# 10XGenomics/lariat

Measured on AMD Instinct MI355X. Metric: read-pairs/sec aligned to hg38 (per-barcode align loop: SMEM seeding + SW + RFA/MAPQ on device); synthetic hg38-scale reference, higher is better.
Workload: dtype u64/i32 (FM-index + integer DP), f64 (RFA scores)

## Files before the change

### lariat_amd/csrc/k_smem4.h

```cpp
#pragma once
#ifndef LH_K1_SLAB_CHUNK
#define LH_K1_SLAB_CHUNK 4
#endif
#include "lh_dev.h"
static_assert((LH_MAXLEN + 2) % LH_K1_SLAB_CHUNK == 0, "a lane's list of LH_MAXLEN + 2 entries is a whole number of chunks");

struct __attribute__((aligned(16))) PEnt { u64 lo, hi; };
#define LH_M40 0xffffffffffull
__device__ __forceinline__ PEnt pe_pack(u64 x0, u64 x1, u64 x2, int info) {
    PEnt e;
    e.lo = x0 | (x2 << 40);
    e.hi = x1 | ((x2 >> 24) << 40) | ((u64)(uint32_t)info << 49);
    return e;
}
#define PE_X0(e) ((e).lo & LH_M40)
#define PE_X1(e) ((e).hi & LH_M40)
#define PE_X2(e) (((e).lo >> 40) | ((((e).hi >> 40) & 0x1ffull) << 24))
#define PE_INFO(e) ((int)((e).hi >> 49))
#define LH_POSF (1ull << 62)

#define S4_FETCH 0
#define S4_DONE 1
#define S4_REQ_FWD 2
#define S4_REQ_BWD 3
// ... 136 lines not shown
#define K1T_BLOOM2 3
#define K1T_REPT 4
#define K1T_PLCP 5
#define K1T_TEXT 6
#define K1T_SA 7
#define K1T_ISA 8
#define K1T_SLAB_R 9
#define K1T_SLAB_W 10
#define K1T_INTV_W 11
#define K1T_READS 12
#define K1T_N 13
#ifdef LH_K1_TRACE
__device__ u64* lh_k1_trace;
__device__ uint32_t lh_k1_trace_cap;
__device__ uint32_t* lh_k1_trace_n;
#define K1_REQ(tab_, ptr_, bytes_)                                                                                                              \
    {                                                                                                                                            \
        if (PASS == 1 && !BIG && lh_k1_trace) {                                                                                                  \
            if (trace_k < lh_k1_trace_cap) lh_k1_trace[(size_t)trace_k * T + t] = (u64)(uintptr_t)(ptr_) | (u64)(bytes_) << 48 | (u64)(tab_) << 56; \
            ++trace_k;                                                                                                                           \
        }                                                                                                                                        \
    }
#else
#define K1_REQ(tab_, ptr_, bytes_)
#endif

template <int PASS, bool BIG>
__global__ void __launch_bounds__(64, PASS == 3 ? 8 : LH_SMEM4_WAVES) k_smem_pass(DIndex ix, DOpts o, int n_reads_all, const uint8_t* __restrict__ seq, const i64* __restrict__ seq_off,
                                               DIntv* __restrict__ intv_out, int32_t* __restrict__ n_intv, int32_t* __restrict__ status, PEnt* __restrict__ slab,
                                               int32_t* __restrict__ next_read, DCounters* __restrict__ ctr, K1Big big) {
    const int n_reads = (BIG || big.list) ? *big.count : n_reads_all;
    constexpr int ICAP = BIG ? LH_BIG_INTV : LH_MAX_INTV;
    __shared__ uint32_t qn[32 * 64];
    constexpr bool DO1 = PASS == 1, DO2 = PASS == 2, DO12 = DO1 || DO2, DO3 = PASS == 3, P3T = PASS == 3;
    const bool P2TASK = PASS == 2 && !BIG && big.list != nullptr;
    int task_k = 0;
    const bool P3TEXT = P3T && ix.isa != nullptr && ix.plcp != nullptr && o.max_mem_intv > 1;
    const int Lw = o.min_seed_len + 1;
    uint32_t uspan = 0;
#define P3_NOTEXT (1 << 30)
    u64 up0 = 0, up1 = 0;
#define US0 ((int)(uspan & 0xff))
#define UE0 ((int)((uspan >> 8) & 0xff))
#define US1 ((int)((uspan >> 16) & 0xff))
#define UE1 ((int)(uspan >> 24))
    const int lane = LANE();
    const uint32_t T = gridDim.x * 64u, t = blockIdx.x * 64u + (uint32_t)lane;
#ifdef LH_K1_TRACE
    uint32_t trace_k = 0;
// ... 39 lines not shown
#define RF_TRIF 128
    int todo = 0;
#define CODE16(s_, out_)                                                                                     \
    {                                                                                                        \
        uint32_t a_, b_;                                                                                     \
        Q8(s_, a_) Q8((s_) + 8, b_)                                                                          \
        a_ &= 0x33333333u; b_ &= 0x33333333u;                                                                \
        a_ = (a_ | a_ >> 2) & 0x0f0f0f0fu; a_ = (a_ | a_ >> 4) & 0x00ff00ffu; a_ = (a_ | a_ >> 8) & 0xffffu; \
        b_ = (b_ | b_ >> 2) & 0x0f0f0f0fu; b_ = (b_ | b_ >> 4) & 0x00ff00ffu; b_ = (b_ | b_ >> 8) & 0xffffu; \
        out_ = a_ | b_ << 16;                                                                                \
    }
#define QB(i_) ((int)((qn[((i_) >> 3) * 64 + lane] >> (((i_) & 7) * 4)) & 0xF))
#define Q8(s_, out_)                                                                                         \
    {                                                                                                        \
        int w_ = (s_) >> 3, sh_ = ((s_) & 7) * 4;                                                            \
        uint32_t lo_ = (w_ >= 0 && w_ < 32) ? qn[w_ * 64 + lane] : 0x44444444u;                              \
        uint32_t hi_ = (w_ + 1 >= 0 && w_ + 1 < 32) ? qn[(w_ + 1) * 64 + lane] : 0x44444444u;                \
        out_ = sh_ ? (lo_ >> sh_) | (hi_ << (32 - sh_)) : lo_;                                               \
    }
#define T16_LOAD(p_) { i64 w_ = (p_) >> 3; tw_sh = (uint32_t)((p_) & 7) * 4; tw0 = ix.tn[w_]; tw1 = ix.tn[w_ + 1]; tw2 = ix.tn[w_ + 2]; K1_REQ(K1T_TEXT, ix.tn + w_, 12) }
#define T16_A() (tw_sh ? (tw0 >> tw_sh) | (tw1 << (32 - tw_sh)) : tw0)
#define T16_B() (tw_sh ? (tw1 >> tw_sh) | (tw2 << (32 - tw_sh)) : tw1)
#define CURR ((rflags & RF_CURA) ? LA : LB)
#define PREV ((rflags & RF_CURA) ? LB : LA)
#define K1_SLAB_IX(e_) (((uint32_t)(e_) / LH_K1_SLAB_CHUNK) * (LH_K1_SLAB_CHUNK * T) + ((uint32_t)(e_) % LH_K1_SLAB_CHUNK))
#define PREV_AT(e_) PREV[K1_SLAB_IX(e_)]
#define FWD_ADVANCE()                                                                                        \
    {                                                                                                        \
        int b_ = i < len ? QB(i) : 4;                                                                        \
        if (b_ > 3) {       \
            ce = pe_pack(c0, c1, c2, cinfo);         \
            ncurr++;                                                                                         \
            st = S4_BWD_INIT;                                                                                \
        } else { ec = 3 - b_; st = S4_REQ_FWD; }                                                             \
    }
#define BLOOM_ISSUE()                                                                                        \
    {                                                                                                        \
        bword = 0; bmask = filt ? 1 : 0;    \
        if (pbits && cinfo - x <= LH_BLOOM_K) bword = (pbits >> (cinfo - x - 1)) & 1;    \
        else if (filt && cinfo >= filt_from) {                                                               \
            uint32_t w_;                                                                                     \
// ... 55 lines not shown
    }
#define BWD_ROW_BODY()                                                                                       \
    {                                                                                                        \
        int c_ = i < 0 ? 4 : QB(i);                                                                          \
        ncurr = 0; last_size = 0; j = 0;                                                                     \
        c0 = PE_X0(ce); c1 = PE_X1(ce); c2 = PE_X2(ce); cinfo = PE_INFO(ce);                                 \
        if (c_ > 3) {                  \
            if ((rflags & (RF_C1UNK | RF_RUNP)) == (RF_C1UNK | RF_RUNP)) { c0 = LH_POSF | (u64)run_p; c1 = 0; }    \
            st = S4_BWD_EMIT0;                                                                               \
        }                                                                                                    \
        else if (runs && nprev == 1 && c2 == 1 && min_intv == 1) { rflags &= ~RF_TRI; st = S4_BRUN_INIT; }    \
          \
        else if (by_text && (rflags & (RF_REV | RF_TRIF)) == RF_REV && nprev > 1 && c2 == 1 && min_intv == 1) { rflags |= RF_TRI; st = S4_BRUN_INIT; } \
        else {                                                                                               \
            ec = c_; st = S4_REQ_BWD;                                                                        \
            if (nprev > 1) { pn = PREV_AT((rflags & RF_REV) ? nprev - 2 : 1); K1_REQ(K1T_SLAB_R, &PREV_AT((rflags & RF_REV) ? nprev - 2 : 1), 16) }                                                \
            if (ktl) CODE16(i, rcode)                                                                        \
        }                                                                                                    \
    }
#define BWD_ADVANCE()                                                                                        \
    {                                                                                                        \
        ++j;                                                                                                 \
        if (j < nprev) {                                                                                     \
            c0 = PE_X0(pn); c1 = PE_X1(pn); c2 = PE_X2(pn); cinfo = PE_INFO(pn);                             \
            st = S4_REQ_BWD;                                                                                 \
            if (j + 1 < nprev) { pn = PREV_AT((rflags & RF_REV) ? nprev - 2 - j : j + 1); K1_REQ(K1T_SLAB_R, &PREV_AT((rflags & RF_REV) ? nprev - 2 - j : j + 1), 16) }                                    \
        } else if (ncurr == 0) st = S4_SMEM_DONE;                                                            \
        else {                                                                                               \
            nprev = ncurr; --i;                                                                              \
            rflags = (rflags ^ RF_CURA) & ~(RF_RUNP | RF_C1UNK | RF_REV);    \
            if (i < -1) st = S4_SMEM_DONE;                                                                   \
            else { todo |= TD_ROW; st = S4_PENDING; }                                                        \
        }                                                                                                    \
    }
#define EMIT_MEM()                                                                                           \
    {                                                                                                        \
        if (cinfo - (i + 1) >= o.min_seed_len) {                                                             \
            DIntv m_; m_.x0 = c0; m_.x1 = c1; m_.x2 = c2; m_.info = (u64)(uint32_t)cinfo | (u64)(i + 1) << 32;  \
            if (P2TASK) {        \
                const int slot_ = atomicAdd(&n_intv[r], 1);                                                  \
                if (slot_ >= ICAP) ovf = 1; else out[slot_] = m_;                                            \
// ... 4 lines not shown
    }
    for (;;) {
        const bool slow_turn = __popcll(__ballot(st == S4_FETCH || (st >= 8 && st < S4_FRUN_INIT))) >= (PASS == 3 ? LH_SLOW_BATCH_P3 : PASS == 2 ? LH_SLOW_BATCH_P2 : LH_SLOW_BATCH) ||
                               !__any((st >= S4_REQ_FWD && st < 8) || st >= S4_FRUN_INIT);
        u64 need = slow_turn ? __ballot(st == S4_FETCH) : 0;
        if (need) {
            int cnt = __popcll(need), newbase = 0;
            if (chunk_next + cnt > chunk_end) {
                int nb = 0;
                if (lane == 0) nb = atomicAdd(next_read, 64);
                newbase = wave_readlane(nb, 0);
            }
            i64 off = 0;
            int ln = 0, rr = -1;
            if (st == S4_FETCH) {
                int idx = chunk_next + lanes_below(need, lane);
                rr = idx < chunk_end ? idx : newbase + (idx - chunk_end);
                if (rr >= n_reads) st = S4_DONE;
                else {
                    if (BIG || big.list) rr = big.list[rr];
                    if (P2TASK) { task_k = rr & 15; rr >>= 4; }
                    off = seq_off[rr]; ln = (int)(seq_off[rr + 1] - off);
                }
            }
            if (chunk_next + cnt > chunk_end) { chunk_next = newbase + (chunk_next + cnt - chunk_end); chunk_end = newbase + 64; }
            else chunk_next += cnt;
            u64 got = __ballot(st == S4_FETCH);
            while (got) {
                int Lk[4], lnk[4];
                uint32_t wk[4];
                for (int k = 0; k < 4; ++k) {
// ... 4 lines not shown
                        const i64 offL = shfl_i64(off, Lk[k]);
                        lnk[k] = wave_readlane(ln, Lk[k]);
                        if (lnk[k] > LH_MAXLEN) lnk[k] = 0;
                        if (4 * lane < lnk[k]) __builtin_memcpy(&wk[k], seq + offL + 4 * lane, 4);
                    }
                }
                for (int k = 0; k < 4; ++k) {
                    if (Lk[k] < 0) break;
                    uint32_t nb16 = 0;
                    for (int b = 0; b < 4; ++b) {
                        uint32_t v = (wk[k] >> (8 * b)) & 0xff;
                        v = (4 * lane + b < lnk[k] && v < 4) ? v : 4;
                        nb16 |= v << (4 * b);
                    }
                    uint32_t other = __shfl_xor(nb16, 1);
                    if (!(lane & 1)) qn[(lane >> 1) * 64 + Lk[k]] = nb16 | other << 16;
                }
            }
            if (st == S4_FETCH) {
                r = rr; len = ln; rst = 0; on = 0; ovf = 0; p2mask = 0; rflags = 0;
                K1_REQ(K1T_READS, seq + off, 64)
                K1_REQ(K1T_READS, seq_off + rr, 16)
                if (len > LH_MAXLEN) { rst |= LH_ST_TOO_LONG; len = 0; }
                out = BIG ? big.slab + (size_t)big.slot[r] * (2 * LH_BIG_INTV) : intv_out + (size_t)r * LH_MAX_INTV;
                if (!DO1) { on = n_intv[r]; rst |= status[r]; }
                if (len >= o.min_seed_len) { x = 0; st = DO1 ? S4_P1_SCAN : DO2 ? S4_P2_NEXT : S4_P3_SCAN; }
                else st = S4_READ_DONE;
                if (DO1 && !BIG && big.resume) {
                    const K1Resume rs = big.resume[r];
                    if (rs.x > 0 && st == S4_P1_SCAN) {
                        x = rs.x; on = n_intv[r]; SET_X_PREV(((rs.pk >> 8) & 0xff) - 2); SET_BT_SKIP(((rs.pk >> 16) & 0xff) - 1);
// ... 312 lines not shown
            const u64 xb = isb ? c1 : c0;
            u64 s0 = tl[0] - tk[0], s1 = tl[1] - tk[1], s2 = tl[2] - tk[2], s3 = tl[3] - tk[3];
            u64 acc = xb + ((xa <= ix.primary && xa + c2 - 1 >= ix.primary) ? 1 : 0);
            u64 o3 = acc, o2 = o3 + s3, o1 = o2 + s2, o0 = o1 + s1;
            u64 na = ec == 0 ? ix.L2[0] + 1 + tk[0] : ec == 1 ? ix.L2[1] + 1 + tk[1] : ec == 2 ? ix.L2[2] + 1 + tk[2] : ix.L2[3] + 1 + tk[3];
            u64 nb = ec == 0 ? o0 : ec == 1 ? o1 : ec == 2 ? o2 : o3;
            ok.x2 = ec == 0 ? s0 : ec == 1 ? s1 : ec == 2 ? s2 : s3;
            if (isb) { ok.x0 = na; ok.x1 = nb; } else { ok.x1 = na; ok.x0 = nb; }
            n_exec_total++;
        }
        if (req) n_ext_total++;
        if (DO12 && st == S4_REQ_FWD) {
            if (ok.x2 != c2) {
                ce = pe_pack(c0, c1, c2, cinfo);
                if (ok.x2 < (u64)min_intv) { st = S4_BWD_INIT; ncurr++; }
                else if (FWD_PUSH_OK()) { if (!ncurr) emin = cinfo; CURR[K1_SLAB_IX(ncurr)] = ce; K1_REQ(K1T_SLAB_W, &CURR[K1_SLAB_IX(ncurr)], 16) ncurr++; }
            }
            if (st == S4_REQ_FWD) {
                c0 = ok.x0; c1 = ok.x1; c2 = ok.x2; cinfo = i + 1; ++i;
                wkey = wkey >> 2 | (u64)(3 - ec) << (2 * LH_BLOOM_K - 2);
                if (runs && c2 == 1 && min_intv == 1) st = S4_FRUN_INIT;
                else { todo |= TD_FADV; st = S4_PENDING; }
            }
        } else if (DO12 && st == S4_REQ_BWD) {
            if (ok.x2 < (u64)min_intv) {
                if (ncurr == 0 && (last_mem_start < 0 || i + 1 < last_mem_start)) st = S4_BWD_EMIT;
            } else if (ncurr == 0 || ok.x2 != last_size) {
                PEnt e = pe_pack(ok.x0, ok.x1, ok.x2, cinfo);
                if (ncurr == 0) ce = e;
                else { CURR[K1_SLAB_IX(ncurr)] = e; K1_REQ(K1T_SLAB_W, &CURR[K1_SLAB_IX(ncurr)], 16) }
                ncurr++;
                last_size = ok.x2;
            }
            if (st == S4_REQ_BWD) BWD_ADVANCE()
        } else if (DO1 && st == S4_REQ_FRUN) {
            uint32_t qa, qb;
            Q8(i, qa)
            Q8(i + 8, qb)
            uint32_t xa = qa ^ T16_A(), xb = qb ^ T16_B();
            int n = xa ? (__ffs((int)xa) - 1) >> 2 : 8 + (xb ? (__ffs((int)xb) - 1) >> 2 : 8);
            if (!(rflags & RF_BT)) n_ext_total += (unsigned)n;
            i += n;
            if (n == 16) T16_LOAD(run_p + (i - x))
            else if (rflags & RF_BT) {
                if (ec < i - x) {
// ... 35 lines not shown
            } else {
                c0 = ok.x0; c1 = ok.x1; c2 = ok.x2; ++i;
                P3_ADVANCE()
            }
        }
    }
#undef QB
#undef Q8
#undef CODE16
#undef T16_LOAD
#undef T16_A
#undef T16_B
#undef CURR
#undef PREV
#undef PREV_AT
#undef K1_SLAB_IX
#undef P3_NOTEXT
#undef US0
#undef UE0
#undef US1
#undef UE1
#undef START_SMEM1
#undef WKEY_AT
#undef BLOOM_ISSUE
#undef FWD_PUSH_OK
#undef FWD_ADVANCE
#undef P3_ADVANCE
#undef BWD_ROW_BODY
#undef BWD_ADVANCE
#undef EMIT_MEM
// ... 37 lines not shown
            const u64 e = trace[(size_t)k * T + t];
            const int tab = (int)(e >> 56), bytes = (int)((e >> 48) & 0xff);
            const uintptr_t a = (uintptr_t)(e & 0xffffffffffffull) + (acc == 0x9e3779b97f4a7c15ull ? 64 : 0);
            if (tab == K1T_SLAB_W) {
                uint4 v = {(uint32_t)acc, 1, 2, 3};
                *(uint4*)a = v;
            } else if (bytes >= 32) { const uint4 v0 = ((const uint4*)a)[0], v1 = ((const uint4*)a)[1]; acc += v0.x + v1.w; }
            else if (bytes >= 16) { const uint4 v = *(const uint4*)a; acc += v.x + v.w; }
            else if (bytes == 12) { const uint32_t* q = (const uint32_t*)a; acc += q[0] + q[1] + q[2]; }
            else if (bytes == 8) acc += *(const u64*)a;
            else acc += *(const uint8_t*)a;
        }
    }
    if (acc == 0x9e3779b97f4a7c15ull) *sink = acc;
}
__global__ void __launch_bounds__(256) k_k1_trace_hist(const u64* __restrict__ trace, const uint32_t* __restrict__ n_req, uint32_t cap, uint32_t T, unsigned long long* __restrict__ hist) {
    __shared__ unsigned long long h[2 * K1T_N + 2];
    if (threadIdx.x < 2 * K1T_N + 2) h[threadIdx.x] = 0;
    __syncthreads();
    for (uint32_t t = blockIdx.x * blockDim.x + threadIdx.x; t < T; t += gridDim.x * blockDim.x) {
        uint32_t n = n_req[t];
        if (n > cap) { atomicAdd(&h[2 * K1T_N], (unsigned long long)(n - cap)); n = cap; }
        for (uint32_t k = 0; k < n; ++k) {
            const u64 e = trace[(size_t)k * T + t];
            const int tab = (int)(e >> 56);
            if (tab < K1T_N) { atomicAdd(&h[2 * tab], 1ull); atomicAdd(&h[2 * tab + 1], (unsigned long long)((e >> 48) & 0xff)); }
        }
    }
    __syncthreads();
    if (threadIdx.x < 2 * K1T_N + 2 && h[threadIdx.x]) atomicAdd(&hist[threadIdx.x], h[threadIdx.x]);
// ... 239 lines not shown
```

### lariat_amd/csrc/lh_host.inc

```
#include <math.h>
#include <stdlib.h>
#include <stdio.h>
#include <string.h>

#include <functional>
#include <memory>
#include <mutex>
#include <string>
#include <vector>
#include <map>

#include "../../include/lariat_hip.h"
#include "k_smem4.h"
#include "k_chain_lane.h"
#include "k_chain_cl.h"
#include "k_rfa.h"
#include "k_rescue3.h"

#define LH_RFA_FIELDS DInf S; uint8_t* d_slab = nullptr; i64 slab_bytes = 0; int grid_rfa = 0; int32_t* d_bc_next = nullptr; \
    uint8_t* d_slab2 = nullptr; i64 slab2_bytes = 0; int grid_rfa2 = 0; uint8_t* d_slab_mid[2] = {nullptr, nullptr}; i64 slab_mid_bytes[2] = {0, 0}; int grid_rfa_mid[2] = {0, 0}; int grid_rfa_mid_max[2] = {0, 0}; int32_t* d_rfa_ovf_mid = nullptr;  int32_t* d_rfa_ovf = nullptr; int32_t* d_rfa_order = nullptr; int32_t *d_rfa_ovf2 = nullptr, *d_rfa_hp = nullptr, *d_rfa_hr = nullptr; double* d_bc_lmp = nullptr;

#define LH_STAGE2_FIELDS                                                                                         \
    i64* d_reg_off = nullptr; DReg* d_regs = nullptr; DReg* d_regs_tmp = nullptr; int32_t* d_ia = nullptr;        \
    int32_t* d_n_regs = nullptr; int32_t* d_best = nullptr; uint8_t* d_zpool = nullptr;                           \
// ... 52 lines not shown
    hipStream_t stream = nullptr;
    hipStream_t aux[3] = {nullptr, nullptr, nullptr};
    hipStream_t dl_stream = nullptr, up_stream = nullptr;
    hipEvent_t ev_pack = nullptr, ev_dl = nullptr;
    bool dl_pending = false, dl_split = false; std::function<int(lh_result**)> dl_finish;
    int sel_slot = 0;
    i64* h_peek = nullptr;
    bool ext_hint_valid = false;
    hipEvent_t ev_fork = nullptr, ev_join[3] = {nullptr, nullptr, nullptr};
    i64 cap_pairs = 0, cap_reads = 0, cap_bases = 0, pool_cap = 0, regpool_cap = 0, cap_bc = 0;
    int grid_smem4 = 0; PEnt* d_slab4 = nullptr; int32_t* d_next_read = nullptr;
    uint32_t* d_seq4 = nullptr;
    uint8_t* d_seq = nullptr; i64* d_seq_off = nullptr; u64* d_name_seed = nullptr; int32_t* d_bc_pair_off = nullptr; uint8_t* d_bc_do_rfa = nullptr;
    i64 *d_cen_start = nullptr, *d_cen_end = nullptr;
    int n_pairs = 0, n_reads = 0, n_bc = 0; bool has_cen = false; i64 n_bases = 0; const uint32_t* q4 = nullptr;
    DIntv* d_intv = nullptr; DIntv* d_big_slab = nullptr; int32_t *d_big_slot = nullptr, *d_big_list = nullptr, *d_big_count = nullptr; int big_cap = 0, big_base = 0;
    K1Resume* d_k1_resume = nullptr; int32_t *d_k1_todo = nullptr, *d_p2_tasks = nullptr;
    int32_t *d_n_intv = nullptr, *d_seed_cnt = nullptr, *d_l_rep = nullptr, *d_status = nullptr;
    i64* d_seed_off = nullptr; DSeed* d_seeds = nullptr; int32_t *d_s_rid = nullptr, *d_s_next = nullptr, *d_ord = nullptr, *d_srt = nullptr;
    DChainTmp* d_ct = nullptr; DChain* d_chains = nullptr; DSeed* d_cseeds = nullptr; int32_t* d_n_chains = nullptr;
    DCounters* d_ctr = nullptr; i64* d_tile_sum = nullptr;
    int32_t* d_wd = nullptr;
    LH_STAGE2_FIELDS
    hipEvent_t ev[LH_NSTAGE + 1];
    const char* tnames[LH_NSTAGE];
    float tms[LH_NSTAGE];
    int n_t = 0;
    bool resident = false, ran = false;
    struct DevBatch {
        uint8_t* seq = nullptr; i64* seq_off = nullptr; u64* name_seed = nullptr; int32_t* bc_pair_off = nullptr; uint8_t* bc_do_rfa = nullptr;
        i64 *cen_start = nullptr, *cen_end = nullptr;
        int n_pairs = 0, n_reads = 0, n_bc = 0; bool has_cen = false, filled = false; i64 n_bases = 0;
        i64 cap_bases = 0; int cap_reads = 0, cap_bc = 0;
    };
    std::vector<DevBatch> slots; std::mutex slot_mu;
    std::vector<void*> free_later;
    lh_context_opts co;
    uint32_t flags = 0;
    std::vector<lh_context*> more;
    std::vector<std::vector<int32_t>> slot_cut;
    int cur_slot = 0;
};

const char* lh_last_error(void) { return g_err.c_str(); }
extern "C" int lh_set_error_(int code, const char* msg) { return set_err(code, msg ? msg : ""); }

int lh_device_count(void) {
// ... 158 lines not shown
    for (int i = 0; i < 3; ++i) { if (c->aux[i]) hipStreamDestroy(c->aux[i]); if (c->ev_join[i]) hipEventDestroy(c->ev_join[i]); }
    if (c->ev_fork) hipEventDestroy(c->ev_fork);
    if (c->dl_pending) { lh_result* r = nullptr; if (c->dl_finish && c->dl_finish(&r) == LH_OK) lh_result_free(r); c->dl_pending = false; }
    if (c->h_peek) hipHostFree(c->h_peek);
    if (c->dl_stream) hipStreamDestroy(c->dl_stream);
    if (c->up_stream) hipStreamDestroy(c->up_stream);
    if (c->ev_pack) hipEventDestroy(c->ev_pack);
    if (c->ev_dl) hipEventDestroy(c->ev_dl);
    if (c->stream) hipStreamDestroy(c->stream);
    delete c;
}

static void select_slot(lh_context* c, const lh_context::DevBatch& sl) {
    c->d_seq = sl.seq; c->d_seq_off = sl.seq_off; c->d_name_seed = sl.name_seed; c->d_bc_pair_off = sl.bc_pair_off; c->d_bc_do_rfa = sl.bc_do_rfa;
    c->d_cen_start = sl.cen_start; c->d_cen_end = sl.cen_end;
    c->n_pairs = sl.n_pairs; c->n_reads = sl.n_reads; c->n_bc = sl.n_bc; c->has_cen = sl.has_cen; c->n_bases = sl.n_bases;
}

static int pipe_upload_slot(lh_context* c, int32_t slot, const lh_batch* b, bool staged) {
    if (!c || !b || !b->seq_off || !b->seq || !b->bc_pair_off) return set_err(LH_E_ARG, "lh_batch_upload: null argument");
    if (slot < 0 || slot > 4096) return set_err(LH_E_ARG, "lh_batch_upload_slot: slot out of range");
    hipStream_t us = staged ? c->up_stream : c->stream;
    if (b->n_pairs <= 0 || b->n_pairs > c->cap_pairs) return set_err(LH_E_CAPACITY, "batch larger than the context capacity");
    if (b->n_barcodes <= 0 || b->n_barcodes > c->cap_bc) return set_err(LH_E_ARG, "bad barcode count");
    if (b->bc_pair_off[0] != 0 || b->bc_pair_off[b->n_barcodes] != b->n_pairs) return set_err(LH_E_ARG, "bc_pair_off must cover [0,n_pairs]");
    HIPCHK(hipSetDevice(c->idx->device));
    int n_reads = 2 * b->n_pairs;
    i64 nb = b->seq_off[n_reads];
    if (nb > c->cap_bases) return set_err(LH_E_CAPACITY, "too many bases for the context");
    if (b->seq_off[0] != 0) return set_err(LH_E_ARG, "seq_off must start at 0");
    for (int r = 0; r < n_reads; ++r) {
        i64 l = b->seq_off[r + 1] - b->seq_off[r];
        if (l < 0) return set_err(LH_E_ARG, "seq_off must be non-decreasing (read " + std::to_string(r) + ")");
        if (l > LH_MAX_READ_LEN) return set_err(LH_E_LIMIT, "read " + std::to_string(r) + " is longer than LH_MAX_READ_LEN");
    }
    for (int k = 0; k < b->n_barcodes; ++k)
        if (b->bc_pair_off[k + 1] < b->bc_pair_off[k]) return set_err(LH_E_ARG, "bc_pair_off must be non-decreasing (barcode " + std::to_string(k) + ")");
    size_t nc = c->idx->names.size();
    lh_context::DevBatch* slp;
    {
        std::lock_guard<std::mutex> g(c->slot_mu);
        if (staged && c->resident && slot == c->sel_slot) return set_err(LH_E_ARG, "lh_batch_stage_slot: that slot is the selected one (stage into another, then lh_batch_select)");
        if ((size_t)slot >= c->slots.size()) c->slots.resize((size_t)slot + 1);
        slp = &c->slots[(size_t)slot];
        slp->filled = false;
    }
    lh_context::DevBatch& sl = *slp;
    if (slot > 0 && (nb > sl.cap_bases || n_reads > sl.cap_reads || b->n_barcodes > sl.cap_bc)) {
        void* old[7] = {sl.seq, sl.seq_off, sl.name_seed, sl.bc_pair_off, sl.bc_do_rfa, sl.cen_start, sl.cen_end};
        if (staged) { std::lock_guard<std::mutex> g(c->slot_mu); for (void* q : old) if (q) c->free_later.push_back(q); }
        else for (void* q : old) hipFree(q);
        sl = lh_context::DevBatch();
        sl.cap_bases = nb + nb / 16; sl.cap_reads = n_reads; sl.cap_bc = b->n_barcodes;
        DALLOC(sl.seq, (size_t)sl.cap_bases + 64); DALLOC(sl.seq_off, (size_t)n_reads + 1); DALLOC(sl.name_seed, (size_t)b->n_pairs);
        DALLOC(sl.bc_pair_off, (size_t)b->n_barcodes + 1); DALLOC(sl.bc_do_rfa, (size_t)b->n_barcodes); DALLOC(sl.cen_start, nc); DALLOC(sl.cen_end, nc);
    }
    sl.n_pairs = b->n_pairs; sl.n_reads = n_reads; sl.n_bc = b->n_barcodes; sl.n_bases = nb;
    HIPCHK(hipMemcpyAsync(sl.seq, b->seq, (size_t)nb, hipMemcpyHostToDevice, us));
    HIPCHK(hipMemcpyAsync(sl.seq_off, b->seq_off, (size_t)(n_reads + 1) * 8, hipMemcpyHostToDevice, us));
    std::vector<u64> seeds;
    const u64* ns = (const u64*)b->name_seed;
    if (!ns) { seeds.assign(b->n_pairs, 1); ns = seeds.data(); }
    HIPCHK(hipMemcpyAsync(sl.name_seed, ns, (size_t)b->n_pairs * 8, hipMemcpyHostToDevice, us));
    HIPCHK(hipMemcpyAsync(sl.bc_pair_off, b->bc_pair_off, (size_t)(b->n_barcodes + 1) * 4, hipMemcpyHostToDevice, us));
    std::vector<uint8_t> rfa;
    const uint8_t* pr = b->bc_do_rfa;
    if (!pr) { rfa.assign(b->n_barcodes, 1); pr = rfa.data(); }
    HIPCHK(hipMemcpyAsync(sl.bc_do_rfa, pr, (size_t)b->n_barcodes, hipMemcpyHostToDevice, us));
    sl.has_cen = b->cen_start && b->cen_end;
    std::vector<i64> neg(nc, -1);
    HIPCHK(hipMemcpyAsync(sl.cen_start, sl.has_cen ? b->cen_start : neg.data(), nc * 8, hipMemcpyHostToDevice, us));
    HIPCHK(hipMemcpyAsync(sl.cen_end, sl.has_cen ? b->cen_end : neg.data(), nc * 8, hipMemcpyHostToDevice, us));
// ... 73 lines not shown
        q4 = c->d_seq4 + 2;
    }
    c->q4 = q4;
    DIndex ix4 = ix;
    if (c->flags & LH_F_NO_SWEEP_FILTER) ix4.bloom1 = ix4.bloom2 = nullptr;
    {
        const int g4 = (N + 63) / 64 < c->grid_smem4 ? (N + 63) / 64 : c->grid_smem4;
        HIPCHK(hipMemsetAsync(c->d_next_read, 0, 8 * sizeof(int32_t), c->stream));
        K1Big nobig; nobig.list = nullptr; nobig.count = nullptr; nobig.slot = nullptr; nobig.slab = nullptr; nobig.resume = nullptr;
        K1Big first = nobig; first.list = c->d_k1_todo; first.count = c->d_next_read + 6; first.resume = c->d_k1_resume;
        const int g3 = (N + 63) / 64 < 2 * c->grid_smem4 ? (N + 63) / 64 : 2 * c->grid_smem4;
        T_BEGIN("k_smem4");
        LH_LAUNCH(k_smem_first, (N + 255) / 256, 256, c->stream, ix4, o, N, q4, (const i64*)c->d_seq_off, c->d_intv, c->d_n_intv, c->d_status, c->d_k1_resume, c->d_k1_todo, c->d_next_read + 6, c->d_ctr);
#ifdef LH_K1_TRACE
        u64* d_trace = nullptr; uint32_t* d_trace_n = nullptr; const uint32_t trace_cap = 4096;
        const bool tracing = getenv("LH_K1_TRACE") != nullptr;
        if (tracing) {
            const size_t Tl = (size_t)g4 * 64;
            DALLOC(d_trace, Tl * trace_cap); DALLOC(d_trace_n, Tl);
            HIPCHK(hipMemsetAsync(d_trace_n, 0, Tl * 4, c->stream));
            HIPCHK(hipMemcpyToSymbolAsync(HIP_SYMBOL(lh_k1_trace), &d_trace, sizeof d_trace, 0, hipMemcpyHostToDevice, c->stream));
            HIPCHK(hipMemcpyToSymbolAsync(HIP_SYMBOL(lh_k1_trace_cap), &trace_cap, sizeof trace_cap, 0, hipMemcpyHostToDevice, c->stream));
            HIPCHK(hipMemcpyToSymbolAsync(HIP_SYMBOL(lh_k1_trace_n), &d_trace_n, sizeof d_trace_n, 0, hipMemcpyHostToDevice, c->stream));
        }
#endif
        LH_LAUNCH((k_smem_pass<1, false>), g4, 64, c->stream, ix4, o, N, c->d_seq, c->d_seq_off, c->d_intv, c->d_n_intv, c->d_status, c->d_slab4, c->d_next_read, c->d_ctr, first);
        T_END();
#ifdef LH_K1_TRACE
        if (tracing) {
            u64* nul = nullptr;
            HIPCHK(hipMemcpyToSymbolAsync(HIP_SYMBOL(lh_k1_trace), &nul, sizeof nul, 0, hipMemcpyHostToDevice, c->stream));
            u64* d_sink = nullptr; unsigned long long* d_hist = nullptr;
            DALLOC(d_sink, 1); DALLOC(d_hist, 2 * K1T_N + 2);
            HIPCHK(hipMemsetAsync(d_hist, 0, (2 * K1T_N + 2) * 8, c->stream));
            hipEvent_t e0, e1;
            HIPCHK(hipEventCreate(&e0)); HIPCHK(hipEventCreate(&e1));
            float best = 1e30f, sum = 0;
            for (int rep_ = 0; rep_ < 4; ++rep_) {
                HIPCHK(hipEventRecord(e0, c->stream));
                LH_LAUNCH(k_k1_replay, g4, 64, c->stream, (const u64*)d_trace, (const uint32_t*)d_trace_n, trace_cap, d_sink);
                HIPCHK(hipEventRecord(e1, c->stream));
                HIPCHK(hipEventSynchronize(e1));
                float ms = 0; HIPCHK(hipEventElapsedTime(&ms, e0, e1));
                if (rep_) { sum += ms; best = ms < best ? ms : best; }
            }
            LH_LAUNCH(k_k1_trace_hist, 2048, 256, c->stream, (const u64*)d_trace, (const uint32_t*)d_trace_n, trace_cap, (uint32_t)(g4 * 64), d_hist);
            unsigned long long h[2 * K1T_N + 2];
            HIPCHK(hipMemcpyAsync(h, d_hist, sizeof h, hipMemcpyDeviceToHost, c->stream));
            HIPCHK(hipStreamSynchronize(c->stream));
            static const char* const tn[K1T_N] = {"occurrence", "tree", "bloom1", "bloom2", "rep_t", "plcp", "text", "sa", "isa", "interval_slab_read", "interval_slab_write", "interval_out_write", "reads"};
            std::string js = "{\"pairs\": " + std::to_string(N / 2) + ", \"lanes\": " + std::to_string((long long)g4 * 64) + ", \"replay_ms_avg\": " + std::to_string(sum / 3) + ", \"replay_ms_min\": " + std::to_string(best) +
                             ", \"dropped_requests\": " + std::to_string(h[2 * K1T_N]) + ", \"requests_by_table\": {";
            for (int i = 0; i < K1T_N; ++i) js += std::string(i ? ", " : "") + "\"" + tn[i] + "\": [" + std::to_string(h[2 * i]) + ", " + std::to_string(h[2 * i + 1]) + "]";
            js += "}}";
            fprintf(stderr, "[lh] K1TRACE %s\n", js.c_str());
            hipEventDestroy(e0); hipEventDestroy(e1);
            hipFree(d_trace); hipFree(d_trace_n); hipFree(d_sink); hipFree(d_hist);
        }
#endif
        T_BEGIN("k_smem4_p2");
        const bool p2_tasks = ((c->flags & LH_F_P2_TASKS) || (c->ext_hint_valid && c->h_peek[4] >= ext_long_min(N))) && N < (1 << 27);
        if (p2_tasks) {
            K1Big p2 = nobig; p2.list = c->d_p2_tasks; p2.count = c->d_next_read + 7; p2.slot = c->d_k1_todo;
            LH_LAUNCH(k_p2_tasks, (N + 255) / 256, 256, c->stream, o, N, (const DIntv*)c->d_intv, (const int32_t*)c->d_n_intv, c->d_p2_tasks, c->d_next_read + 7, c->d_k1_todo);
            LH_LAUNCH((k_smem_pass<2, false>), g4, 64, c->stream, ix4, o, N, c->d_seq, c->d_seq_off, c->d_intv, c->d_n_intv, c->d_status, c->d_slab4, c->d_next_read + 1, c->d_ctr, p2);
            LH_LAUNCH(k_p2_clamp, (N + 255) / 256, 256, c->stream, N, c->d_n_intv);
        } else
        LH_LAUNCH((k_smem_pass<2, false>), g4, 64, c->stream, ix4, o, N, c->d_seq, c->d_seq_off, c->d_intv, c->d_n_intv, c->d_status, c->d_slab4, c->d_next_read + 1, c->d_ctr, nobig);
        T_END();
        T_BEGIN("k_smem4_p3");
        if (o.max_mem_intv > 0 && q4)
            LH_LAUNCH(k_smem_p3_lock, (N + 255) / 256, 256, c->stream, ix4, o, N, q4, (const i64*)c->d_seq_off, c->d_intv, c->d_n_intv, c->d_status, c->d_ctr);
        else if (o.max_mem_intv > 0)
            LH_LAUNCH((k_smem_pass<3, false>), g3, 64, c->stream, ix4, o, N, c->d_seq, c->d_seq_off, c->d_intv, c->d_n_intv, c->d_status, c->d_slab4, c->d_next_read + 2, c->d_ctr, nobig);
        T_END();
        T_BEGIN("k_smem_fin");
        { int rc = k1_big_round(c, o, ix4, N, 0); if (rc) return rc; }
        LH_LAUNCH(k_smem_fin, (N * 16 + 255) / 256, 256, c->stream, o, N, c->d_intv, c->d_n_intv, c->d_seed_cnt, c->d_l_rep, (const int32_t*)c->d_big_slot);
        T_END();
    }
    T_BEGIN("k_scan_seeds");
    { int rc = run_scan(c, N, c->d_seed_cnt, 0, 0, c->d_seed_off); if (rc) return rc; }
    T_END();
    {
// ... 222 lines not shown
```

Before: 49.06 million.

## Keep the first SMEM interval list entries in an LDS ring

The per-lane interval lists for passes 1 and 2 now keep their first R entries in LDS words placed after the query staging buffer, and only spill to the global slab beyond that. R is sized from a fixed per-block LDS budget. When every read in the batch fits, a smaller query-staging template width is selected so the ring can be larger. The goal is to cut global slab reads and writes during backward extension, at the cost of more LDS traffic and template variants. Tracing also gains list-length histograms and per-table skip replay, and lane indexing switches to mbcnt intrinsics.

```diff
diff --git a/lariat_amd/csrc/k_smem4.h b/lariat_amd/csrc/k_smem4.h
--- a/lariat_amd/csrc/k_smem4.h
+++ b/lariat_amd/csrc/k_smem4.h
@@ -4,6 +4,16 @@
 #endif
 #include "lh_dev.h"
 static_assert((LH_MAXLEN + 2) % LH_K1_SLAB_CHUNK == 0, "a lane's list of LH_MAXLEN + 2 entries is a whole number of chunks");
+#define LH_K1_LDS_BUDGET 10240
+#ifndef LH_K1_QW_SMALL
+#define LH_K1_QW_SMALL 24
+#endif
+#ifdef LH_K1_RING
+#define LH_K1_RING_OF(qw_) (LH_K1_RING)
+#else
+#define LH_K1_RING_OF(qw_) ((LH_K1_LDS_BUDGET - (qw_) * 256) / 2048)
+#endif
+static_assert(LH_K1_QW_SMALL >= 1 && LH_K1_QW_SMALL <= 32, "the small query staging holds at most the full query");
 
 struct __attribute__((aligned(16))) PEnt { u64 lo, hi; };
 #define LH_M40 0xffffffffffull
@@ -174,6 +184,14 @@
 __device__ u64* lh_k1_trace;
 __device__ uint32_t lh_k1_trace_cap;
 __device__ uint32_t* lh_k1_trace_n;
+#define K1L_PUSH 0
+#define K1L_NPREV 1
+#define K1L_READ 2
+__device__ unsigned long long* lh_k1_lens;
+#define K1_LEN(kind_, v_)                                                                                                                        \
+    {                                                                                                                                            \
+        if (DO12 && !BIG && lh_k1_lens) { const int v__ = (v_); atomicAdd(&lh_k1_lens[((PASS - 1) * 3 + (kind_)) * 64 + (v__ < 63 ? v__ : 63)], 1ull); } \
+    }
 #define K1_REQ(tab_, ptr_, bytes_)                                                                                                              \
     {                                                                                                                                            \
         if (PASS == 1 && !BIG && lh_k1_trace) {                                                                                                  \
@@ -183,16 +201,23 @@
     }
 #else
 #define K1_REQ(tab_, ptr_, bytes_)
+#define K1_LEN(kind_, v_)
 #endif
 
-template <int PASS, bool BIG>
+template <int PASS, bool BIG, int QW = 32>
 __global__ void __launch_bounds__(64, PASS == 3 ? 8 : LH_SMEM4_WAVES) k_smem_pass(DIndex ix, DOpts o, int n_reads_all, const uint8_t* __restrict__ seq, const i64* __restrict__ seq_off,
                                                DIntv* __restrict__ intv_out, int32_t* __restrict__ n_intv, int32_t* __restrict__ status, PEnt* __restrict__ slab,
                                                int32_t* __restrict__ next_read, DCounters* __restrict__ ctr, K1Big big) {
     const int n_reads = (BIG || big.list) ? *big.count : n_reads_all;
     constexpr int ICAP = BIG ? LH_BIG_INTV : LH_MAX_INTV;
-    __shared__ uint32_t qn[32 * 64];
     constexpr bool DO1 = PASS == 1, DO2 = PASS == 2, DO12 = DO1 || DO2, DO3 = PASS == 3, P3T = PASS == 3;
+    static_assert(QW >= 1 && QW <= 32, "query staging: 1 to 32 words per lane");
+    constexpr int R = DO12 ? LH_K1_RING_OF(QW) : 0;
+    static_assert(R >= 0, "ring size");
+#ifndef LH_K1_RING
+    static_assert(!DO12 || QW * 256 + R * 2048 <= LH_K1_LDS_BUDGET, "query + ring within the LDS of a block at LH_SMEM4_WAVES waves per SIMD");
+#endif
+    __shared__ uint32_t qn[(QW + 8 * R) * 64];
     const bool P2TASK = PASS == 2 && !BIG && big.list != nullptr;
     int task_k = 0;
     const bool P3TEXT = P3T && ix.isa != nullptr && ix.plcp != nullptr && o.max_mem_intv > 1;
@@ -262,8 +287,8 @@
 #define Q8(s_, out_)                                                                                         \
     {                                                                                                        \
         int w_ = (s_) >> 3, sh_ = ((s_) & 7) * 4;                                                            \
-        uint32_t lo_ = (w_ >= 0 && w_ < 32) ? qn[w_ * 64 + lane] : 0x44444444u;                              \
-        uint32_t hi_ = (w_ + 1 >= 0 && w_ + 1 < 32) ? qn[(w_ + 1) * 64 + lane] : 0x44444444u;                \
+        uint32_t lo_ = (w_ >= 0 && w_ < QW) ? qn[w_ * 64 + lane] : 0x44444444u;                              \
+        uint32_t hi_ = (w_ + 1 >= 0 && w_ + 1 < QW) ? qn[(w_ + 1) * 64 + lane] : 0x44444444u;                \
         out_ = sh_ ? (lo_ >> sh_) | (hi_ << (32 - sh_)) : lo_;                                               \
     }
 #define T16_LOAD(p_) { i64 w_ = (p_) >> 3; tw_sh = (uint32_t)((p_) & 7) * 4; tw0 = ix.tn[w_]; tw1 = ix.tn[w_ + 1]; tw2 = ix.tn[w_ + 2]; K1_REQ(K1T_TEXT, ix.tn + w_, 12) }
@@ -273,6 +298,25 @@
 #define PREV ((rflags & RF_CURA) ? LB : LA)
 #define K1_SLAB_IX(e_) (((uint32_t)(e_) / LH_K1_SLAB_CHUNK) * (LH_K1_SLAB_CHUNK * T) + ((uint32_t)(e_) % LH_K1_SLAB_CHUNK))
 #define PREV_AT(e_) PREV[K1_SLAB_IX(e_)]
+#define RING_W(a_, p_) (&qn[(QW + 4 * (((a_) ? 0 : R) + (p_))) * 64 + lane])
+#define LIST_PUT(p_, e_)                                                                                     \
+    {                                                                                                        \
+        const int p__ = (p_);                                                                                \
+        K1_LEN(K1L_PUSH, ncurr)                                                                              \
+        if ((unsigned)p__ < (unsigned)R) {                                                                   \
+            uint32_t* w_ = RING_W(rflags & RF_CURA, p__);                                                    \
+            w_[0] = (uint32_t)(e_).lo; w_[64] = (uint32_t)((e_).lo >> 32); w_[128] = (uint32_t)(e_).hi; w_[192] = (uint32_t)((e_).hi >> 32); \
+        } else { CURR[K1_SLAB_IX(p__)] = (e_); K1_REQ(K1T_SLAB_W, &CURR[K1_SLAB_IX(p__)], 16) }              \
+    }
+#define LIST_GET(p_, out_)                                                                                   \
+    {                                                                                                        \
+        const int p__ = (p_);                                                                                \
+        K1_LEN(K1L_NPREV, nprev) K1_LEN(K1L_READ, p__)                                                       \
+        if ((unsigned)p__ < (unsigned)R) {                                                                   \
+            const uint32_t* w_ = RING_W(!(rflags & RF_CURA), p__);                                           \
+            out_.lo = (u64)w_[0] | (u64)w_[64] << 32; out_.hi = (u64)w_[128] | (u64)w_[192] << 32;           \
+        } else { out_ = PREV_AT(p__); K1_REQ(K1T_SLAB_R, &PREV_AT(p__), 16) }                                \
+    }
 #define FWD_ADVANCE()                                                                                        \
     {                                                                                                        \
         int b_ = i < len ? QB(i) : 4;                                                                        \
@@ -358,7 +402,7 @@
         else if (by_text && (rflags & (RF_REV | RF_TRIF)) == RF_REV && nprev > 1 && c2 == 1 && min_intv == 1) { rflags |= RF_TRI; st = S4_BRUN_INIT; } \
         else {                                                                                               \
             ec = c_; st = S4_REQ_BWD;                                                                        \
-            if (nprev > 1) { pn = PREV_AT((rflags & RF_REV) ? nprev - 2 : 1); K1_REQ(K1T_SLAB_R, &PREV_AT((rflags & RF_REV) ? nprev - 2 : 1), 16) }                                                \
+            if (nprev > 1) LIST_GET((rflags & RF_REV) ? nprev - 2 : 0, pn)                                  \
             if (ktl) CODE16(i, rcode)                                                                        \
         }                                                                                                    \
     }
@@ -368,7 +412,7 @@
         if (j < nprev) {                                                                                     \
             c0 = PE_X0(pn); c1 = PE_X1(pn); c2 = PE_X2(pn); cinfo = PE_INFO(pn);                             \
             st = S4_REQ_BWD;                                                                                 \
-            if (j + 1 < nprev) { pn = PREV_AT((rflags & RF_REV) ? nprev - 2 - j : j + 1); K1_REQ(K1T_SLAB_R, &PREV_AT((rflags & RF_REV) ? nprev - 2 - j : j + 1), 16) }                                    \
+            if (j + 1 < nprev) LIST_GET((rflags & RF_REV) ? nprev - 2 - j : j, pn)                           \
         } else if (ncurr == 0) st = S4_SMEM_DONE;                                                            \
         else {                                                                                               \
             nprev = ncurr; --i;                                                                              \
@@ -403,7 +447,11 @@
             i64 off = 0;
             int ln = 0, rr = -1;
             if (st == S4_FETCH) {
+#ifdef LH_EMU
                 int idx = chunk_next + lanes_below(need, lane);
+#else
+                int idx = chunk_next + (int)__builtin_amdgcn_mbcnt_hi((uint32_t)(need >> 32), __builtin_amdgcn_mbcnt_lo((uint32_t)need, 0u));
+#endif
                 rr = idx < chunk_end ? idx : newbase + (idx - chunk_end);
                 if (rr >= n_reads) st = S4_DONE;
                 else {
@@ -438,7 +486,7 @@
                         nb16 |= v << (4 * b);
                     }
                     uint32_t other = __shfl_xor(nb16, 1);
-                    if (!(lane & 1)) qn[(lane >> 1) * 64 + Lk[k]] = nb16 | other << 16;
+                    if (!(lane & 1) && (lane >> 1) < QW) qn[(lane >> 1) * 64 + Lk[k]] = nb16 | other << 16;
                 }
             }
             if (st == S4_FETCH) {
@@ -781,7 +829,7 @@
             if (ok.x2 != c2) {
                 ce = pe_pack(c0, c1, c2, cinfo);
                 if (ok.x2 < (u64)min_intv) { st = S4_BWD_INIT; ncurr++; }
-                else if (FWD_PUSH_OK()) { if (!ncurr) emin = cinfo; CURR[K1_SLAB_IX(ncurr)] = ce; K1_REQ(K1T_SLAB_W, &CURR[K1_SLAB_IX(ncurr)], 16) ncurr++; }
+                else if (FWD_PUSH_OK()) { if (!ncurr) emin = cinfo; LIST_PUT(ncurr, ce) ncurr++; }
             }
             if (st == S4_REQ_FWD) {
                 c0 = ok.x0; c1 = ok.x1; c2 = ok.x2; cinfo = i + 1; ++i;
@@ -795,7 +843,7 @@
             } else if (ncurr == 0 || ok.x2 != last_size) {
                 PEnt e = pe_pack(ok.x0, ok.x1, ok.x2, cinfo);
                 if (ncurr == 0) ce = e;
-                else { CURR[K1_SLAB_IX(ncurr)] = e; K1_REQ(K1T_SLAB_W, &CURR[K1_SLAB_IX(ncurr)], 16) }
+                else LIST_PUT(ncurr - 1, e)
                 ncurr++;
                 last_size = ok.x2;
             }
@@ -861,6 +909,9 @@
 #undef CURR
 #undef PREV
 #undef PREV_AT
+#undef RING_W
+#undef LIST_PUT
+#undef LIST_GET
 #undef K1_SLAB_IX
 #undef P3_NOTEXT
 #undef US0
@@ -928,6 +979,17 @@
     }
     if (acc == 0x9e3779b97f4a7c15ull) *sink = acc;
 }
+__global__ void __launch_bounds__(256) k_k1_trace_skip(u64* __restrict__ trace, uint32_t* __restrict__ n_req, uint32_t cap, uint32_t T, uint32_t skip_mask) {
+    for (uint32_t t = blockIdx.x * blockDim.x + threadIdx.x; t < T; t += gridDim.x * blockDim.x) {
+        uint32_t n = n_req[t], w = 0;
+        if (n > cap) n = cap;
+        for (uint32_t k = 0; k < n; ++k) {
+            const u64 e = trace[(size_t)k * T + t];
+            if (!((skip_mask >> (int)(e >> 56)) & 1u)) trace[(size_t)(w++) * T + t] = e;
+        }
+        n_req[t] = w;
+    }
+}
 __global__ void __launch_bounds__(256) k_k1_trace_hist(const u64* __restrict__ trace, const uint32_t* __restrict__ n_req, uint32_t cap, uint32_t T, unsigned long long* __restrict__ hist) {
     __shared__ unsigned long long h[2 * K1T_N + 2];
     if (threadIdx.x < 2 * K1T_N + 2) h[threadIdx.x] = 0;
diff --git a/lariat_amd/csrc/lh_host.inc b/lariat_amd/csrc/lh_host.inc
--- a/lariat_amd/csrc/lh_host.inc
+++ b/lariat_amd/csrc/lh_host.inc
@@ -90,6 +90,7 @@
     uint8_t* d_seq = nullptr; i64* d_seq_off = nullptr; u64* d_name_seed = nullptr; int32_t* d_bc_pair_off = nullptr; uint8_t* d_bc_do_rfa = nullptr;
     i64 *d_cen_start = nullptr, *d_cen_end = nullptr;
     int n_pairs = 0, n_reads = 0, n_bc = 0; bool has_cen = false; i64 n_bases = 0; const uint32_t* q4 = nullptr;
+    int max_len = LH_MAXLEN;
     DIntv* d_intv = nullptr; DIntv* d_big_slab = nullptr; int32_t *d_big_slot = nullptr, *d_big_list = nullptr, *d_big_count = nullptr; int big_cap = 0, big_base = 0;
     K1Resume* d_k1_resume = nullptr; int32_t *d_k1_todo = nullptr, *d_p2_tasks = nullptr;
     int32_t *d_n_intv = nullptr, *d_seed_cnt = nullptr, *d_l_rep = nullptr, *d_status = nullptr;
@@ -106,7 +107,7 @@
     struct DevBatch {
         uint8_t* seq = nullptr; i64* seq_off = nullptr; u64* name_seed = nullptr; int32_t* bc_pair_off = nullptr; uint8_t* bc_do_rfa = nullptr;
         i64 *cen_start = nullptr, *cen_end = nullptr;
-        int n_pairs = 0, n_reads = 0, n_bc = 0; bool has_cen = false, filled = false; i64 n_bases = 0;
+        int n_pairs = 0, n_reads = 0, n_bc = 0; bool has_cen = false, filled = false; i64 n_bases = 0; int max_len = LH_MAXLEN;
         i64 cap_bases = 0; int cap_reads = 0, cap_bc = 0;
     };
     std::vector<DevBatch> slots; std::mutex slot_mu;
@@ -295,7 +296,7 @@
 static void select_slot(lh_context* c, const lh_context::DevBatch& sl) {
     c->d_seq = sl.seq; c->d_seq_off = sl.seq_off; c->d_name_seed = sl.name_seed; c->d_bc_pair_off = sl.bc_pair_off; c->d_bc_do_rfa = sl.bc_do_rfa;
     c->d_cen_start = sl.cen_start; c->d_cen_end = sl.cen_end;
-    c->n_pairs = sl.n_pairs; c->n_reads = sl.n_reads; c->n_bc = sl.n_bc; c->has_cen = sl.has_cen; c->n_bases = sl.n_bases;
+    c->n_pairs = sl.n_pairs; c->n_reads = sl.n_reads; c->n_bc = sl.n_bc; c->has_cen = sl.has_cen; c->n_bases = sl.n_bases; c->max_len = sl.max_len;
 }
 
 static int pipe_upload_slot(lh_context* c, int32_t slot, const lh_batch* b, bool staged) {
@@ -310,10 +311,12 @@
     i64 nb = b->seq_off[n_reads];
     if (nb > c->cap_bases) return set_err(LH_E_CAPACITY, "too many bases for the context");
     if (b->seq_off[0] != 0) return set_err(LH_E_ARG, "seq_off must start at 0");
+    i64 lmax = 0;
     for (int r = 0; r < n_reads; ++r) {
         i64 l = b->seq_off[r + 1] - b->seq_off[r];
         if (l < 0) return set_err(LH_E_ARG, "seq_off must be non-decreasing (read " + std::to_string(r) + ")");
         if (l > LH_MAX_READ_LEN) return set_err(LH_E_LIMIT, "read " + std::to_string(r) + " is longer than LH_MAX_READ_LEN");
+        lmax = l > lmax ? l : lmax;
     }
     for (int k = 0; k < b->n_barcodes; ++k)
         if (b->bc_pair_off[k + 1] < b->bc_pair_off[k]) return set_err(LH_E_ARG, "bc_pair_off must be non-decreasing (barcode " + std::to_string(k) + ")");
@@ -336,7 +339,7 @@
         DALLOC(sl.seq, (size_t)sl.cap_bases + 64); DALLOC(sl.seq_off, (size_t)n_reads + 1); DALLOC(sl.name_seed, (size_t)b->n_pairs);
         DALLOC(sl.bc_pair_off, (size_t)b->n_barcodes + 1); DALLOC(sl.bc_do_rfa, (size_t)b->n_barcodes); DALLOC(sl.cen_start, nc); DALLOC(sl.cen_end, nc);
     }
-    sl.n_pairs = b->n_pairs; sl.n_reads = n_reads; sl.n_bc = b->n_barcodes; sl.n_bases = nb;
+    sl.n_pairs = b->n_pairs; sl.n_reads = n_reads; sl.n_bc = b->n_barcodes; sl.n_bases = nb; sl.max_len = (int)lmax;
     HIPCHK(hipMemcpyAsync(sl.seq, b->seq, (size_t)nb, hipMemcpyHostToDevice, us));
     HIPCHK(hipMemcpyAsync(sl.seq_off, b->seq_off, (size_t)(n_reads + 1) * 8, hipMemcpyHostToDevice, us));
     std::vector<u64> seeds;
@@ -440,17 +443,22 @@
         LH_LAUNCH(k_smem_first, (N + 255) / 256, 256, c->stream, ix4, o, N, q4, (const i64*)c->d_seq_off, c->d_intv, c->d_n_intv, c->d_status, c->d_k1_resume, c->d_k1_todo, c->d_next_read + 6, c->d_ctr);
 #ifdef LH_K1_TRACE
         u64* d_trace = nullptr; uint32_t* d_trace_n = nullptr; const uint32_t trace_cap = 4096;
+        unsigned long long* d_lens = nullptr;
         const bool tracing = getenv("LH_K1_TRACE") != nullptr;
         if (tracing) {
             const size_t Tl = (size_t)g4 * 64;
-            DALLOC(d_trace, Tl * trace_cap); DALLOC(d_trace_n, Tl);
+            DALLOC(d_trace, Tl * trace_cap); DALLOC(d_trace_n, Tl); DALLOC(d_lens, 2 * 3 * 64);
             HIPCHK(hipMemsetAsync(d_trace_n, 0, Tl * 4, c->stream));
+            HIPCHK(hipMemsetAsync(d_lens, 0, 2 * 3 * 64 * 8, c->stream));
+            HIPCHK(hipMemcpyToSymbolAsync(HIP_SYMBOL(lh_k1_lens), &d_lens, sizeof d_lens, 0, hipMemcpyHostToDevice, c->stream));
             HIPCHK(hipMemcpyToSymbolAsync(HIP_SYMBOL(lh_k1_trace), &d_trace, sizeof d_trace, 0, hipMemcpyHostToDevice, c->stream));
             HIPCHK(hipMemcpyToSymbolAsync(HIP_SYMBOL(lh_k1_trace_cap), &trace_cap, sizeof trace_cap, 0, hipMemcpyHostToDevice, c->stream));
             HIPCHK(hipMemcpyToSymbolAsync(HIP_SYMBOL(lh_k1_trace_n), &d_trace_n, sizeof d_trace_n, 0, hipMemcpyHostToDevice, c->stream));
         }
 #endif
-        LH_LAUNCH((k_smem_pass<1, false>), g4, 64, c->stream, ix4, o, N, c->d_seq, c->d_seq_off, c->d_intv, c->d_n_intv, c->d_status, c->d_slab4, c->d_next_read, c->d_ctr, first);
+        const bool qw_small = c->max_len <= 8 * LH_K1_QW_SMALL;
+        if (qw_small) LH_LAUNCH((k_smem_pass<1, false, LH_K1_QW_SMALL>), g4, 64, c->stream, ix4, o, N, c->d_seq, c->d_seq_off, c->d_intv, c->d_n_intv, c->d_status, c->d_slab4, c->d_next_read, c->d_ctr, first);
+        else LH_LAUNCH((k_smem_pass<1, false>), g4, 64, c->stream, ix4, o, N, c->d_seq, c->d_seq_off, c->d_intv, c->d_n_intv, c->d_status, c->d_slab4, c->d_next_read, c->d_ctr, first);
         T_END();
 #ifdef LH_K1_TRACE
         if (tracing) {
@@ -461,24 +469,42 @@
             HIPCHK(hipMemsetAsync(d_hist, 0, (2 * K1T_N + 2) * 8, c->stream));
             hipEvent_t e0, e1;
             HIPCHK(hipEventCreate(&e0)); HIPCHK(hipEventCreate(&e1));
+            auto replay = [&](float& best, float& sum) -> int {
+                best = 1e30f; sum = 0;
+                for (int rep_ = 0; rep_ < 4; ++rep_) {
+                    HIPCHK(hipEventRecord(e0, c->stream));
+                    LH_LAUNCH(k_k1_replay, g4, 64, c->stream, (const u64*)d_trace, (const uint32_t*)d_trace_n, trace_cap, d_sink);
+                    HIPCHK(hipEventRecord(e1, c->stream));
+                    HIPCHK(hipEventSynchronize(e1));
+                    float ms = 0; HIPCHK(hipEventElapsedTime(&ms, e0, e1));
+                    if (rep_) { sum += ms; best = ms < best ? ms : best; }
+                }
+                return LH_OK;
+            };
             float best = 1e30f, sum = 0;
-            for (int rep_ = 0; rep_ < 4; ++rep_) {
-                HIPCHK(hipEventRecord(e0, c->stream));
-                LH_LAUNCH(k_k1_replay, g4, 64, c->stream, (const u64*)d_trace, (const uint32_t*)d_trace_n, trace_cap, d_sink);
-                HIPCHK(hipEventRecord(e1, c->stream));
-                HIPCHK(hipEventSynchronize(e1));
-                float ms = 0; HIPCHK(hipEventElapsedTime(&ms, e0, e1));
-                if (rep_) { sum += ms; best = ms < best ? ms : best; }
-            }
+            { int rc = replay(best, sum); if (rc) return rc; }
             LH_LAUNCH(k_k1_trace_hist, 2048, 256, c->stream, (const u64*)d_trace, (const uint32_t*)d_trace_n, trace_cap, (uint32_t)(g4 * 64), d_hist);
             unsigned long long h[2 * K1T_N + 2];
             HIPCHK(hipMemcpyAsync(h, d_hist, sizeof h, hipMemcpyDeviceToHost, c->stream));
             HIPCHK(hipStreamSynchronize(c->stream));
+            std::string skip_js;
+            if (const char* sk = getenv("LH_K1_REPLAY_SKIP")) {
+                for (const char* q = sk; *q;) {
+                    char* end = nullptr;
+                    const unsigned long m = strtoul(q, &end, 0);
+                    if (end == q) break;
+                    LH_LAUNCH(k_k1_trace_skip, 2048, 256, c->stream, d_trace, d_trace_n, trace_cap, (uint32_t)(g4 * 64), (uint32_t)m);
+                    float b_ = 0, s_ = 0;
+                    { int rc = replay(b_, s_); if (rc) return rc; }
+                    skip_js += std::string(skip_js.empty() ? "" : ", ") + "{\"skip_mask\": " + std::to_string(m) + ", \"replay_ms_avg\": " + std::to_string(s_ / 3) + ", \"replay_ms_min\": " + std::to_string(b_) + "}";
+                    q = *end == ',' ? end + 1 : end;
+                }
+            }
             static const char* const tn[K1T_N] = {"occurrence", "tree", "bloom1", "bloom2", "rep_t", "plcp", "text", "sa", "isa", "interval_slab_read", "interval_slab_write", "interval_out_write", "reads"};
             std::string js = "{\"pairs\": " + std::to_string(N / 2) + ", \"lanes\": " + std::to_string((long long)g4 * 64) + ", \"replay_ms_avg\": " + std::to_string(sum / 3) + ", \"replay_ms_min\": " + std::to_string(best) +
                              ", \"dropped_requests\": " + std::to_string(h[2 * K1T_N]) + ", \"requests_by_table\": {";
             for (int i = 0; i < K1T_N; ++i) js += std::string(i ? ", " : "") + "\"" + tn[i] + "\": [" + std::to_string(h[2 * i]) + ", " + std::to_string(h[2 * i + 1]) + "]";
-            js += "}}";
+            js += "}, \"replay_without\": [" + skip_js + "]}";
             fprintf(stderr, "[lh] K1TRACE %s\n", js.c_str());
             hipEventDestroy(e0); hipEventDestroy(e1);
             hipFree(d_trace); hipFree(d_trace_n); hipFree(d_sink); hipFree(d_hist);
@@ -489,11 +515,34 @@
         if (p2_tasks) {
             K1Big p2 = nobig; p2.list = c->d_p2_tasks; p2.count = c->d_next_read + 7; p2.slot = c->d_k1_todo;
             LH_LAUNCH(k_p2_tasks, (N + 255) / 256, 256, c->stream, o, N, (const DIntv*)c->d_intv, (const int32_t*)c->d_n_intv, c->d_p2_tasks, c->d_next_read + 7, c->d_k1_todo);
-            LH_LAUNCH((k_smem_pass<2, false>), g4, 64, c->stream, ix4, o, N, c->d_seq, c->d_seq_off, c->d_intv, c->d_n_intv, c->d_status, c->d_slab4, c->d_next_read + 1, c->d_ctr, p2);
+            if (qw_small) LH_LAUNCH((k_smem_pass<2, false, LH_K1_QW_SMALL>), g4, 64, c->stream, ix4, o, N, c->d_seq, c->d_seq_off, c->d_intv, c->d_n_intv, c->d_status, c->d_slab4, c->d_next_read + 1, c->d_ctr, p2);
+            else LH_LAUNCH((k_smem_pass<2, false>), g4, 64, c->stream, ix4, o, N, c->d_seq, c->d_seq_off, c->d_intv, c->d_n_intv, c->d_status, c->d_slab4, c->d_next_read + 1, c->d_ctr, p2);
             LH_LAUNCH(k_p2_clamp, (N + 255) / 256, 256, c->stream, N, c->d_n_intv);
-        } else
+        } else if (qw_small)
+        LH_LAUNCH((k_smem_pass<2, false, LH_K1_QW_SMALL>), g4, 64, c->stream, ix4, o, N, c->d_seq, c->d_seq_off, c->d_intv, c->d_n_intv, c->d_status, c->d_slab4, c->d_next_read + 1, c->d_ctr, nobig);
+        else
         LH_LAUNCH((k_smem_pass<2, false>), g4, 64, c->stream, ix4, o, N, c->d_seq, c->d_seq_off, c->d_intv, c->d_n_intv, c->d_status, c->d_slab4, c->d_next_read + 1, c->d_ctr, nobig);
         T_END();
+#ifdef LH_K1_TRACE
+        if (tracing) {
+            unsigned long long* nul = nullptr;
+            HIPCHK(hipMemcpyToSymbolAsync(HIP_SYMBOL(lh_k1_lens), &nul, sizeof nul, 0, hipMemcpyHostToDevice, c->stream));
+            unsigned long long hl[2 * 3 * 64];
+            HIPCHK(hipMemcpyAsync(hl, d_lens, sizeof hl, hipMemcpyDeviceToHost, c->stream));
+            HIPCHK(hipStreamSynchronize(c->stream));
+            static const char* const kn[3] = {"ncurr_at_push", "nprev_at_read", "stored_position_read"};
+            std::string js = "{";
+            for (int ps = 0; ps < 2; ++ps)
+                for (int k = 0; k < 3; ++k) {
+                    js += std::string(ps || k ? ", " : "") + "\"pass" + std::to_string(ps + 1) + "_" + kn[k] + "\": [";
+                    for (int v = 0; v < 64; ++v) js += std::string(v ? ", " : "") + std::to_string(hl[(ps * 3 + k) * 64 + v]);
+                    js += "]";
+                }
+            js += "}";
+            fprintf(stderr, "[lh] K1LENS %s\n", js.c_str());
+            hipFree(d_lens);
+        }
+#endif
         T_BEGIN("k_smem4_p3");
         if (o.max_mem_intv > 0 && q4)
             LH_LAUNCH(k_smem_p3_lock, (N + 255) / 256, 256, c->stream, ix4, o, N, q4, (const i64*)c->d_seq_off, c->d_intv, c->d_n_intv, c->d_status, c->d_ctr);
```

Measured after the change: 49.85 million, median of 6. 1.6% higher.
